# lms-org/trajectory_controller

Measured on AMD Instinct MI355X. Metric: MPC QP solves/sec (horizon N=20, 2 inputs) at 1/2/4/8 MI355X; max|du| vs dlib, higher is better.
Workload: dtype f64; 1 GPU; batch 262144 trajectories per GPU, N=20, 2 inputs, compact (mpcControllerTobi) form, cold start, eps 0.01, max_iter 10000; global_batch=262144, horizon=20, algo=lane_fma, parallelism=batch-sharded x1, batches_in_flight=1, gather=none (1 GPU)

## Files before the change

trajectory_controller_amd/csrc/mpc_internal.h:

```cpp
#pragma once

#include <hip/hip_runtime.h>
#include <stdint.h>

namespace tpc {

constexpr int kWave = 64;

struct Knobs {
    double eps;
    uint32_t max_iter;
    uint32_t smo_iters;
};

struct CompactArgs {
    int64_t n;
    const void *v, *dy, *dphi;
    void *front, *rear;
    int32_t* iters;
    uint32_t* flags;
    const int32_t* work_hint;
    double step, wheelbase;
    double q[2], r[2], lo[2], hi[2];
    int table_key;
// ... 25 lines not shown
struct Workspace {
    void* state;
    uint32_t* ticket;
    unsigned long long* stats;
    int64_t capacity_bytes;
    uint32_t *keys, *rank, *order;
    void* sort_temp;
    size_t sort_temp_bytes;
    hipEvent_t* ev;
    int wave_group = 0;
    int group_lanes = 0;
    int max_waves = 0;
    bool group_pair = false;
    int64_t lanex_below = -1;
    int cu_count = 0;
};

constexpr int kQueueTickets = 16;
constexpr int kQueueTicketStride = 64;
constexpr int64_t kQueueTicketBytes = (int64_t)kQueueTickets * kQueueTicketStride * 4;
constexpr int64_t kWaveQueueMaxInstances = 32768;

constexpr int kAlgoMixed = 101;
constexpr int kAlgoGeneric = 100;
constexpr int kMaxHorizon = 64;
int64_t generic_scratch_bytes(int H, int dtype, int64_t n);
hipError_t generic_compact(int dtype, int H, const CompactArgs& a, const Knobs& k, void* scratch, hipStream_t s);
hipError_t generic_general(int dtype, int I, int H, const GeneralArgs& a, const Knobs& k, void* scratch, hipStream_t s);

size_t sort_temp_bytes(int64_t n);
hipError_t order_begin(void* temp, hipStream_t s);
hipError_t presolve_merge(const uint32_t* queue, const uint32_t* queue_len, int64_t n, const void* sf, const void* sr,
                          const int32_t* si, void* f, void* r, int32_t* it, uint32_t limit, hipStream_t s);
hipError_t presolve_merge_rows(const uint32_t* queue, const uint32_t* queue_len, int64_t n, const void* su, const int32_t* si,
                               void* u, int32_t* it, int rows, int64_t ld, uint32_t limit, hipStream_t s);
const uint32_t* order_queue_len(const void* temp);
hipError_t order_finish(const uint32_t* keys, const uint32_t* rank, uint32_t* order, int64_t n, void* temp,
                        hipStream_t s);

struct RolloutStepArgs {
    int64_t n, ld, ld_out, ld_nlt;
    int I, H, step, steps;
    const void *A, *B, *C;
    void* x;
    void* targets;
// ... 40 lines not shown
```

trajectory_controller_amd/csrc/mpc_lane_inst.hip:

```cpp
#include <cstdint>

#include "mpc_lane.h"
#include "mpc_lanex.h"

#ifndef TPC_LANE_H
#error "compile with -DTPC_LANE_H=<horizon>"
#endif

namespace tpc {

namespace {

constexpr int kH = TPC_LANE_H;

template <class Tag, class Kernel>
inline int pg_grid(Kernel kernel, int block) {
    constexpr int kMaxDev = 64;
    static int cache[kMaxDev] = {0};
    int dev = 0;
    if (hipGetDevice(&dev) != hipSuccess) dev = 0;
    if (dev >= 0 && dev < kMaxDev && cache[dev] > 0) return cache[dev];
    int cus = 256, per_cu = 4;
    hipDeviceProp_t prop;
    if (hipGetDeviceProperties(&prop, dev) == hipSuccess) cus = prop.multiProcessorCount;
    if (hipOccupancyMaxActiveBlocksPerMultiprocessor(&per_cu, kernel, block, 0) != hipSuccess || per_cu < 1)
        per_cu = 1;
    if (per_cu > 4) per_cu = 4;
    if (dev >= 0 && dev < kMaxDev) cache[dev] = cus * per_cu;
    return cus * per_cu;
}
struct TagState {}; struct TagFast {}; struct TagExact {}; struct TagLanex {}; template <int I> struct TagLanexG {};

inline bool wants_state(const CompactArgs&) { return false; }
inline bool wants_state(const GeneralArgs& a) { return a.controls != nullptr || a.v != nullptr; }

template <typename T, int I, class Model, class Args>
hipError_t phase1(const Args& a, const Knobs& k, const Workspace& ws, hipStream_t s) {
    T* recs = (T*)ws.state;
    hipError_t e = hipMemsetAsync(ws.ticket, 0, sizeof(uint32_t), s);
    if (e == hipSuccess) e = hipMemsetAsync(ws.stats, 0, 3 * sizeof(unsigned long long), s);
    if (e == hipSuccess) e = order_begin(ws.sort_temp, s);
    if (e != hipSuccess) return e;
    const int cd_grid = (int)((a.n + kWave - 1) / kWave);
    if (ws.ev) (void)hipEventRecord(ws.ev[0], s);
    hipLaunchKernelGGL((lane_cd_kernel<T, I, kH, Model, Args>), dim3(cd_grid), dim3(kWave), 0, s, a, k, recs,
                       ws.keys, ws.rank, (uint32_t*)ws.sort_temp, ws.stats, wants_state(a) ? 0 : 1);
    e = hipGetLastError();
    if (e != hipSuccess) return e;
    e = order_finish(ws.keys, ws.rank, ws.order, a.n, ws.sort_temp, s);
    if (e != hipSuccess) return e;
    if (ws.ev) (void)hipEventRecord(ws.ev[1], s);
    return hipSuccess;
}
template <typename T, int I, class Model, class Args>
hipError_t phase2(const Args& a, const Knobs& k, const Workspace& ws, hipStream_t s, bool only_if_refused) {
    T* recs = (T*)ws.state;
// ... 68 lines not shown
            if (ws.ev) (void)hipEventRecord(ws.ev[2], s);
            return e;
        }
    }
    e = phase2<T, I, Model, Args>(a, k, ws, s, false);
    if (ws.ev) (void)hipEventRecord(ws.ev[2], s);
    return e;
}

template <typename T, int I, class Model, class Args, int SUBSET = 1>
hipError_t resolve(const Args& a, const Knobs& k, const Workspace& ws, const int32_t* select, const uint32_t* gate, hipStream_t s,
                   double lambda_from = 0.0, const uint32_t* pre_len = nullptr, uint32_t pre_limit = 0u) {
    if (a.n <= 0) return hipSuccess;
    T* recs = (T*)ws.state;
    uint32_t* queue_len = ws.ticket + 1;
    hipError_t e = hipMemsetAsync(ws.ticket, 0, 32, s);
    if (e != hipSuccess) return e;
    const int grid = (int)((a.n + kWave - 1) / kWave);
    hipLaunchKernelGGL((lane_cd_kernel<T, I, kH, Model, Args, SUBSET>), dim3(grid), dim3(kWave), 0, s, a, k, recs, ws.order,
                       (uint32_t*)nullptr, queue_len, ws.stats, 1, select, gate, (T)lambda_from, pre_len, pre_limit);
    if constexpr (std::is_same<Model, CompactModel<T>>::value && sizeof(T) == 8 && LanexPlan<kH>::built) {
        constexpr int ng = LanexPlan<kH>::NG;
        const int64_t need = (a.n + ng - 1) / ng;
        if constexpr (SUBSET == 2) {
            const int64_t solo = (int64_t)pre_limit / ng;
            hipLaunchKernelGGL((lanex_pg_kernel<T, kH, true>), dim3((unsigned)(need < solo ? need : solo)), dim3(kWave), 0, s, a, k,
                               (const T*)recs, (const uint32_t*)ws.order, ws.ticket, ws.stats, (const uint32_t*)queue_len, 1, pre_limit);
            return hipGetLastError();
        }
        const int grid_cap = pg_grid<TagLanex>(lanex_pg_kernel<T, kH>, kWave);
        hipLaunchKernelGGL((lanex_pg_kernel<T, kH>), dim3((unsigned)(need < grid_cap ? need : grid_cap)), dim3(kWave), 0, s, a, k,
// ... 89 lines not shown
```

trajectory_controller_amd/csrc/mpc_sort.hip:

```cpp
#include "mpc_internal.h"

namespace tpc {

namespace {

constexpr int kBins = 1 << 16;

constexpr int kScanBlocks = 64, kScanThreads = 256, kPerThread = kBins / kScanBlocks / kScanThreads;

__global__ __launch_bounds__(kScanThreads) void scan_sums_kernel(const uint32_t* __restrict__ hist,
                                                                 uint32_t* __restrict__ block_sum) {
    __shared__ uint32_t part[kScanThreads / 64];
    const int t = threadIdx.x;
    const int top = kBins - 1 - (blockIdx.x * kScanThreads + t) * kPerThread;
    uint32_t sum = 0;
    for (int j = 0; j < kPerThread; ++j) sum += hist[top - j];
    for (int off = 32; off > 0; off >>= 1) sum += __shfl_down(sum, off);
    if ((t & 63) == 0) part[t >> 6] = sum;
    __syncthreads();
    if (t == 0) {
        uint32_t tot = 0;
        for (int w = 0; w < kScanThreads / 64; ++w) tot += part[w];
        block_sum[blockIdx.x] = tot;
    }
}

__global__ __launch_bounds__(kScanThreads) void scan_apply_kernel(uint32_t* __restrict__ hist,
                                                                  const uint32_t* __restrict__ block_sum) {
    __shared__ uint32_t part[kScanThreads];
    const int t = threadIdx.x;
    const int top = kBins - 1 - (blockIdx.x * kScanThreads + t) * kPerThread;
    uint32_t c[kPerThread], sum = 0;
    for (int j = 0; j < kPerThread; ++j) { c[j] = hist[top - j]; sum += c[j]; }
    part[t] = sum;
    __syncthreads();
    for (int off = 1; off < kScanThreads; off <<= 1) {
        const uint32_t add = t >= off ? part[t - off] : 0u;
        __syncthreads();
        part[t] += add;
        __syncthreads();
    }
    uint32_t base = part[t] - sum;
    for (int b = 0; b < (int)blockIdx.x; ++b) base += block_sum[b];
    for (int j = 0; j < kPerThread; ++j) {
        hist[top - j] = base;
        base += c[j];
    }
}

__global__ void scatter_kernel(const uint32_t* __restrict__ keys, const uint32_t* __restrict__ rank,
                               const uint32_t* __restrict__ base, uint32_t* __restrict__ order, int64_t n) {
    for (int64_t i = (int64_t)blockIdx.x * blockDim.x + threadIdx.x; i < n; i += (int64_t)gridDim.x * blockDim.x)
        order[base[keys[i] >> 16] + rank[i]] = (uint32_t)i;
}

}

size_t sort_temp_bytes(int64_t) { return (size_t)(kBins + kScanBlocks) * sizeof(uint32_t); }

const uint32_t* order_queue_len(const void* temp) { return (const uint32_t*)temp + 127; }

hipError_t order_begin(void* temp, hipStream_t s) {
    return hipMemsetAsync(temp, 0, (size_t)kBins * sizeof(uint32_t), s);
}

hipError_t order_finish(const uint32_t* keys, const uint32_t* rank, uint32_t* order, int64_t n, void* temp,
                        hipStream_t s) {
    uint32_t* hist = (uint32_t*)temp;
    const int block = 256;
    int64_t g = (n + block - 1) / block;
    const unsigned grid = (unsigned)(g < 2048 ? g : 2048);
    uint32_t* block_sum = hist + kBins;
    hipLaunchKernelGGL(scan_sums_kernel, dim3(kScanBlocks), dim3(kScanThreads), 0, s, (const uint32_t*)hist, block_sum);
    hipLaunchKernelGGL(scan_apply_kernel, dim3(kScanBlocks), dim3(kScanThreads), 0, s, hist, (const uint32_t*)block_sum);
    hipLaunchKernelGGL(scatter_kernel, dim3(grid), dim3(block), 0, s, keys, rank, (const uint32_t*)hist, order, n);
    return hipGetLastError();
}

template <typename T>
__global__ void presolve_merge_kernel(const uint32_t* __restrict__ queue, const uint32_t* __restrict__ queue_len,
                                      const T* __restrict__ sf, const T* __restrict__ sr, const int32_t* __restrict__ si,
                                      T* __restrict__ f, T* __restrict__ r, int32_t* __restrict__ it, uint32_t limit) {
    const uint32_t nq = *queue_len;
    if (nq > limit) return;
    for (uint32_t q = blockIdx.x * blockDim.x + threadIdx.x; q < nq; q += gridDim.x * blockDim.x) {
        const uint32_t k = queue[q];
        f[k] = sf[k];
        r[k] = sr[k];
        if (it) it[k] = si[k];
    }
// ... 29 lines not shown
```

trajectory_controller_amd/csrc/mpc_ub.h:

```cpp
#pragma once

#include "mpc_lane.h"
#include "mpc_ub_model.h"
#include "mpc_ub_cd_asm.h"
#include "mpc_queue_key.h"

namespace tpc {

template <typename T, bool EQB> TPC_DEV void ub_set_uniform(ub::Unit<T, EQB>& m, T gscale, const CompactArgs& g) {
    const T q[2] = {(T)g.q[0], (T)g.q[1]}, r[2] = {(T)g.r[0], (T)g.r[1]};
    const T lo[2] = {(T)g.lo[0], (T)g.lo[1]}, hi[2] = {(T)g.hi[0], (T)g.hi[1]};
    m.set_uniform(gscale, q, r, lo, hi);
}

template <typename T, int H> struct UbCdPlan {
    static constexpr bool mirror = 2 * (2 * H * kWave * (int)sizeof(T)) <= 64 * 1024 &&
                                   2 * (2 * H * kWave * (int)sizeof(T)) * 4 * CdOcc<T, H>::value <= 160 * 1024;
    static constexpr bool x_in_lds = mirror && sizeof(T) == 8 && H >= 20;
    static constexpr bool fast = true;
};

template <typename T, int H, bool EQB> struct UbCdAsm {
#ifdef TPC_UB_CD_NO_ASM
    static constexpr bool value = false;
// ... 2 lines not shown
#endif
};

TPC_DEV double cd_ldexp(double x, int e) { return __builtin_ldexp(x, e); }
TPC_DEV float cd_ldexp(float x, int e) { return __builtin_ldexpf(x, e); }

template <typename T, int H, bool EQB>
__global__ __launch_bounds__(64, (CdOcc<T, H>::value)) void ub_cd_kernel(CompactArgs g, Knobs kn, T* __restrict__ recs,
                                                                         uint32_t* __restrict__ keys,
                                                                         uint32_t* __restrict__ key_rank,
                                                                         uint32_t* __restrict__ key_hist,
                                                                         unsigned long long* __restrict__ stats) {
    using P = UbCdPlan<T, H>;
    constexpr int RL = LaneRec<T, H>::kLen;
    constexpr bool MIRROR = P::mirror, XL = P::x_in_lds;
    __shared__ T s_cd[2 * H + (MIRROR ? 2 * H : 1)][kWave];
    T (*const s_iqd)[kWave] = s_cd;
    T (*const s_x)[kWave] = s_cd + 2 * H;
    const int lane = threadIdx.x;
    const int64_t k = (int64_t)blockIdx.x * kWave + lane;
    if (k >= g.n) return;

    ub::Unit<T, EQB> m;
    ub_set_uniform(m, (T)1, g);
    const T ty = ((const T*)g.dy)[k], tphi = ((const T*)g.dphi)[k];
    const T tv = ((const T*)g.v)[k];
    m.set_instance((T)g.step, (T)g.wheelbase, tv, ty, tphi);
    const bool nonfinite = m.nonfinite_inputs(ty, tphi);
    float table_lf = 0.0f;
    if constexpr (sizeof(T) == 8 && H == kQueueKeyH) {
        const float c = queue_key_predict((double)tv, (double)ty, (double)tphi);
        table_lf = (c * c) * (c * c);
    }
    const T q0 = (T)g.q[0], q1 = (T)g.q[1], r0 = (T)g.r[0], r1 = (T)g.r[1];

    T x[XL ? 1 : 2 * H], w[ub::Reverse<T, H>::value ? 1 : 2 * H];
// ... 100 lines not shown
        } else {
#pragma unroll 1
            for (uint32_t it = 0; it < cd_iters; ++it) {
                if (__ballot(!stopped) == 0ull) break;
                iteration(std::true_type{}, it);
            }
        }
    } else {
#pragma unroll 1
        for (uint32_t it = 0; it < cd_iters; ++it) {
            if (__ballot(!stopped) == 0ull) break;
            iteration(std::false_type{}, it);
        }
    }

    T* rec = recs + (int64_t)k * RL;
#pragma unroll
    for (int q = 0; q < 2 * H; ++q) rec[q] = X(q);
    rec[2 * H] = lambda;
    uint64_t meta = (uint64_t)iter;
    if (stopped) meta |= kMetaStopped;
    if (vinit) meta |= kMetaVInit;
    if (nonfinite) meta |= kMetaNonFinite;
    store_meta<T>(rec + 2 * H + 1, meta);
    {
        T il0, il1, beta;
        ub::pg_constants<T>(lambda, m.s0, m.s1, il0, il1, beta);
        T* ex = rec + LaneRec<T, H>::kExtra;
        ex[0] = il0; ex[1] = il1; ex[2] = beta; ex[3] = m.a; ex[4] = m.c; ex[5] = ty; ex[6] = tphi;
    }
    const bool finished = stopped || iter >= kn.max_iter;
    const T lambda_floor = (r0 + r1) * (T)H;
    const bool uninformative = lambda < (T)1.5 * lambda_floor;
    float lf = (float)lambda;
    if constexpr (sizeof(T) == 8 && H == kQueueKeyH) {
        if (g.table_key) lf = table_lf;
    }
    if (g.work_hint) lf = (float)(g.work_hint[k] > 0 ? g.work_hint[k] : 1);
    const uint32_t spread = (uint32_t)k & 127u;
    uint32_t key = __float_as_uint(lf);
    if (finished) key = spread << 16;
    else if (!g.work_hint && uninformative) key = (0x7f00u + spread) << 16;
    else if (!(lf > 0.0f) || key < 0x00800000u) key = 0x00800000u;
    else if (key >= 0x7f000000u) key = 0x7effffffu;
    uint32_t f = 0;
    if (finished) {
        ((T*)g.front)[k] = nonfinite ? (T)0 : m.control(0, X(0));
        ((T*)g.rear)[k] = nonfinite ? (T)0 : m.control(1, X(1));
        if (g.iters) g.iters[k] = (int32_t)iter;
        if (nonfinite) f |= 0x1u;
        if (!stopped) f |= 0x2u;
    }
    raise_flags(g.flags, f);
    keys[k] = key;
    key_rank[k] = atomicAdd(&key_hist[key >> 16], 1u);
}

#ifndef TPC_UB_OCC
#define TPC_UB_OCC 0
#endif
#ifndef TPC_UB_KV
#define TPC_UB_KV -1
#endif
template <typename T, int H> struct UbPlan {
    static constexpr bool D = sizeof(T) == 8;
    static constexpr int words = D ? 2 : 1;
    static constexpr bool reverse = ub::Reverse<T, H>::value;
    static constexpr bool regs = 6 * H * words <= 200 || !D || (reverse && 4 * H * words <= 200);
// ... 238 lines not shown
```

trajectory_controller_amd/csrc/mpc_ub_inst.hip:

```cpp
#include <cstdint>
#include <type_traits>

#include "mpc_ub.h"

#ifndef TPC_UB_H
#error "compile with -DTPC_UB_H=<horizon>"
#endif

namespace tpc {

hipError_t ub_pg_asm_launch(const CompactArgs& a, const Knobs& k, const Workspace& ws, int64_t need, hipStream_t s);
hipError_t ub_pg_asm_launch_h10(const CompactArgs& a, const Knobs& k, const Workspace& ws, int64_t need, hipStream_t s);

namespace {

constexpr int kH = TPC_UB_H;

template <class Tag, class Kernel>
inline int ub_grid(Kernel kernel, int block) {
    constexpr int kMaxDev = 64;
    static int cache[kMaxDev] = {0};
    int dev = 0;
    if (hipGetDevice(&dev) != hipSuccess) dev = 0;
    if (dev >= 0 && dev < kMaxDev && cache[dev] > 0) return cache[dev];
    int cus = 256, per_cu = 4;
    hipDeviceProp_t prop;
    if (hipGetDeviceProperties(&prop, dev) == hipSuccess) cus = prop.multiProcessorCount;
    if (hipOccupancyMaxActiveBlocksPerMultiprocessor(&per_cu, kernel, block, 0) != hipSuccess || per_cu < 1)
        per_cu = 1;
    if (per_cu > 4) per_cu = 4;
    if (dev >= 0 && dev < kMaxDev) cache[dev] = cus * per_cu;
    return cus * per_cu;
}
template <typename T, bool EQB, int MODE> struct TagPg {};

template <typename T, bool EQB>
hipError_t phase1(const CompactArgs& a, const Knobs& k, const Workspace& ws, hipStream_t s) {
    T* recs = (T*)ws.state;
    hipError_t e = hipMemsetAsync(ws.ticket, 0, sizeof(uint32_t), s);
    if (e == hipSuccess) e = hipMemsetAsync(ws.stats, 0, 3 * sizeof(unsigned long long), s);
    if (e == hipSuccess) e = order_begin(ws.sort_temp, s);
    if (e != hipSuccess) return e;
    const int cd_grid = (int)((a.n + kWave - 1) / kWave);
    if (ws.ev) (void)hipEventRecord(ws.ev[0], s);
    hipLaunchKernelGGL((ub_cd_kernel<T, kH, EQB>), dim3(cd_grid), dim3(kWave), 0, s, a, k, recs, ws.keys, ws.rank,
                       (uint32_t*)ws.sort_temp, ws.stats);
    e = hipGetLastError();
    if (e != hipSuccess) return e;
    e = order_finish(ws.keys, ws.rank, ws.order, a.n, ws.sort_temp, s);
    if (e != hipSuccess) return e;
    if (ws.ev) (void)hipEventRecord(ws.ev[1], s);
    return hipSuccess;
}
template <typename T, bool EQB, int MODE>
hipError_t pg_launch(const CompactArgs& a, const Knobs& k, const Workspace& ws, hipStream_t s) {
    constexpr int bt = kWave * UbPlan<T, kH>::occ;
// ... 58 lines not shown
```

trajectory_controller_amd/csrc/tpc_mpc_api.cpp:

```cpp
#include "tpc_mpc_context.h"
#include "tpc_mpc_experimental.h"
#include "auto_table.h"
#include "mpc_queue_key_table.h"
#include "mpc_grad_model.h"
#include "mpc_polish_model.h"
#include "mpc_rollout_newton.h"
#include "mpc_newton_compact.h"
#include "mpc_tangent_model.h"

#include <cmath>
#include <cstdlib>
#include <mutex>
#include <vector>

namespace tpc {
#define TPC_DECL_H(h)                                                                             \
    hipError_t lane_compact_h##h(int, const CompactArgs&, const Knobs&, const Workspace&, hipStream_t); \
    hipError_t lane_general_h##h(int, int, const GeneralArgs&, const Knobs&, const Workspace&, hipStream_t); \
    hipError_t lane_resolve_compact_h##h(const CompactArgs&, const Knobs&, const Workspace&, const int32_t*, const uint32_t*, hipStream_t, double, const uint32_t*, uint32_t); \
    hipError_t lane_presolve_compact_h##h(const CompactArgs&, const Knobs&, const Workspace&, double, uint32_t, hipStream_t); \
    hipError_t lane_resolve_general_h##h(int, const GeneralArgs&, const Knobs&, const Workspace&, const int32_t*, const uint32_t*, hipStream_t, double, const uint32_t*, uint32_t); \
    hipError_t lane_presolve_general_h##h(int, const GeneralArgs&, const Knobs&, const Workspace&, double, uint32_t, hipStream_t); \
    hipError_t wave_compact_h##h(int, const CompactArgs&, const Knobs&, const Workspace&, hipStream_t); \
    hipError_t wave_general_h##h(int, int, const GeneralArgs&, const Knobs&, const Workspace&, hipStream_t); \
// ... 291 lines not shown
        int rc = ensure(h, &h->ws_state, &h->ws_bytes, pad256(generic_scratch_bytes(H, dtype, n)));
        if (rc) return rc;
        ws->state = h->ws_state;
        ws->capacity_bytes = h->ws_bytes;
    }
    if (algo == TPC_MPC_ALGO_WAVE) {
        int rc = ensure(h, &h->ws_state, &h->ws_bytes, pad256(n * 4) + kQueueTicketBytes);
        if (rc) return rc;
        ws->order = (uint32_t*)h->ws_state;
        ws->ticket = (uint32_t*)((char*)h->ws_state + pad256(n * 4));
        ws->capacity_bytes = h->ws_bytes;
    }
    if (algo == TPC_MPC_ALGO_LANE || algo == TPC_MPC_ALGO_LANE_FMA || algo == TPC_MPC_ALGO_GROUP) {
        const int64_t rec_b = pad256(lane_rec_len(H, dtype) * (int64_t)esize(dtype) * n);
        const int64_t col_b = pad256(n * 4);
        const size_t tmp_b = sort_temp_bytes(n);
        int rc = ensure(h, &h->ws_state, &h->ws_bytes, rec_b + 3 * col_b + pad256((int64_t)tmp_b));
        if (rc) return rc;
        char* b = (char*)h->ws_state;
        ws->state = b;
        ws->keys = (uint32_t*)(b + rec_b);
        ws->rank = (uint32_t*)(b + rec_b + col_b);
        ws->order = (uint32_t*)(b + rec_b + 2 * col_b);
        ws->sort_temp = b + rec_b + 3 * col_b;
        ws->sort_temp_bytes = tmp_b;
        ws->capacity_bytes = h->ws_bytes;
    }
    return TPC_MPC_OK;
}

int resolve_reserve(tpc_mpc_context* h, int H, int dtype, int64_t n) { return reserve_lane_workspace(h, H, dtype, n); }
int resolve_workspace(tpc_mpc_context* h, int H, int dtype, int64_t n, Workspace* ws) {
    const bool ev_valid = h->ev_valid;
    const int last_algo = h->last_algo;
    const int rc = prepare_workspace(h, TPC_MPC_ALGO_LANE, H, dtype, n, ws);
    h->ev_valid = ev_valid;
    h->last_algo = last_algo;
    ws->ev = nullptr;
    ws->ticket = h->ws_words + 16;
    ws->stats = (unsigned long long*)(h->ws_words + 18);
    return rc;
}

hipError_t copy_rows(void* dst, int64_t dpitch, const void* src, int64_t spitch, int64_t width, int64_t rows,
                     hipMemcpyKind kind, hipStream_t s) {
    if (rows <= 0 || width <= 0) return hipSuccess;
    if (dpitch == width && spitch == width) return hipMemcpyAsync(dst, src, (size_t)(width * rows), kind, s);
    return hipMemcpy2DAsync(dst, (size_t)dpitch, src, (size_t)spitch, (size_t)width, (size_t)rows, kind, s);
}

int check_general_io(tpc_mpc_context* h, const tpc_mpc_general_io* io, int mem) {
    if (!io) return fail(h, TPC_MPC_ERR_BAD_ARG, "null io");
    if (io->inputs != 1 && io->inputs != 2) return fail(h, TPC_MPC_ERR_BAD_ARG, "inputs must be 1 or 2");
    if (io->n < 0 || io->ld < io->n || io->n > 0x7fffffffll)
        return fail(h, TPC_MPC_ERR_BAD_ARG, "need 0 <= n <= ld, n < 2^31");
// ... 27 lines not shown

int check_compact_model(tpc_mpc_context* h, const tpc_mpc_params* p) {
    if (!(p->weight_y >= 0) || !(p->weight_phi >= 0))
        return fail(h, TPC_MPC_ERR_BAD_WEIGHTS, "min(Q) >= 0 violated (mpc_abstract.h:90-97)");
    if (!(p->weight_steering_front > 0) || !(p->weight_steering_rear > 0))
        return fail(h, TPC_MPC_ERR_BAD_WEIGHTS, "min(R) > 0 violated (mpc_abstract.h:90-97)");
    for (int j = 0; j < 2; ++j)
        if (!(p->upper[j] >= p->lower[j]))
            return fail(h, TPC_MPC_ERR_BAD_BOUNDS, "upper >= lower violated (mpc_abstract.h:90-97)");
    if (!std::isfinite(p->step_size) || !std::isfinite(p->wheelbase) || p->wheelbase == 0)
        return fail(h, TPC_MPC_ERR_BAD_ARG, "step_size / wheelbase must be finite, wheelbase != 0");
    return TPC_MPC_OK;
}

int stream_order_begin(tpc_mpc_context* h, hipStream_t s) {
    if (h->have_last && h->last_stream != s) HIP_TRY(h, hipStreamWaitEvent(s, h->done_ev, 0));
    return TPC_MPC_OK;
}
int stream_order_end(tpc_mpc_context* h, hipStream_t s) {
    HIP_TRY(h, hipEventRecord(h->done_ev, s));
    h->last_stream = s;
    h->have_last = true;
    return TPC_MPC_OK;
}

int finish_flags(tpc_mpc_context* h, uint32_t* flags_out, hipStream_t s) {
    if (!flags_out) return TPC_MPC_OK;
    uint32_t f = 0;
    HIP_TRY(h, hipMemcpyAsync(&f, h->ws_words + 1, sizeof(f), hipMemcpyDeviceToHost, s));
    HIP_TRY(h, hipStreamSynchronize(s));
    *flags_out = f;
    return TPC_MPC_OK;
}

int reserve_lane_workspace(tpc_mpc_context* h, int H, int dtype, int64_t n) {
    const bool ev_valid = h->ev_valid;
    const int last_algo = h->last_algo;
    Workspace ws;
    const int rc = prepare_workspace(h, horizon_specialised(H) ? TPC_MPC_ALGO_LANE : kAlgoGeneric, H, dtype, n, &ws);
    h->ev_valid = ev_valid;
    h->last_algo = last_algo;
    return rc;
}

int context_new(int device, int cu_count, tpc_mpc_context** out) {
    tpc_mpc_context* h = new (std::nothrow) tpc_mpc_context;
    if (!h) return fail(nullptr, TPC_MPC_ERR_ALLOC, "out of host memory");
    h->device = device;
    h->cu_count = cu_count;
    h->device_cu_count = cu_count;
    hipError_t e = hipSetDevice(device);
    if (e == hipSuccess) e = hipMalloc((void**)&h->ws_words, 128);
    if (e == hipSuccess) e = hipMemset(h->ws_words, 0, 128);
    if (e == hipSuccess) e = hipHostMalloc(&h->pin_host, 512, hipHostMallocMapped | hipHostMallocCoherent);
    if (e == hipSuccess) e = hipHostGetDevicePointer(&h->pin_dev, h->pin_host, 0);
    if (e == hipSuccess) e = hipEventCreateWithFlags(&h->done_ev, hipEventDisableTiming);
    if (e != hipSuccess) {
        (void)tpc_mpc_destroy(h);
        return fail(nullptr, TPC_MPC_ERR_HIP, "create: %s", hipGetErrorString(e));
    }
    std::memset(h->pin_host, 0, 512);
    *out = h;
    return TPC_MPC_OK;
}

static double presolve_lambda(const tpc_mpc_params* p);
static int presolve_scratch(tpc_mpc_context* h, int H, int dtype, int64_t n, int64_t side_bytes, Workspace* ws, char** side) {
    const int64_t rec_b = pad256(lane_rec_len(H, dtype) * (int64_t)esize(dtype) * n), col_b = pad256(n * 4);
// ... 4 lines not shown
    if (!h->pre_stream) HIP_TRY(h, hipStreamCreateWithFlags(&h->pre_stream, hipStreamNonBlocking));
    if (!h->pre_fork) HIP_TRY(h, hipEventCreateWithFlags(&h->pre_fork, hipEventDisableTiming));
    if (!h->pre_done) HIP_TRY(h, hipEventCreateWithFlags(&h->pre_done, hipEventDisableTiming));
    char* b = (char*)h->pre;
    std::memset(ws, 0, sizeof(*ws));
    ws->state = b;
    ws->keys = (uint32_t*)(b + rec_b);
    ws->rank = (uint32_t*)(b + rec_b + col_b);
    ws->order = (uint32_t*)(b + rec_b + 2 * col_b);
    ws->sort_temp = b + rec_b + 3 * col_b;
    ws->sort_temp_bytes = tmp_b;
    ws->capacity_bytes = lane_b;
    ws->ev = nullptr;
    ws->lanex_below = h->opt_lanex_below;
    ws->cu_count = h->cu_count;
    ws->ticket = h->ws_words + 24;
    ws->stats = (unsigned long long*)(h->ws_words + 26);
    *side = b + lane_b;
    return TPC_MPC_OK;
}
static bool presolve_share(tpc_mpc_context* h, int64_t n, Presolve* ps) {
    const int simds = (h->device_cu_count > 0 ? h->device_cu_count : 256) * 4;
    const int solo_waves = simds * 7 / 16;
    if (n > (int64_t)solo_waves * 8 * 5) return false;
    ps->limit = (uint32_t)solo_waves * 8u;
    ps->group_waves = simds - solo_waves;
    return true;
}

int general_launch(tpc_mpc_context* h, const tpc_mpc_params* p, const tpc_mpc_general_io* io, hipStream_t s) {
    const int I = io->inputs, H = p->horizon;
    const int64_t n = io->n;
// ... 180 lines not shown
    if (algo < 0) return fail(h, TPC_MPC_ERR_BAD_HORIZON, "the WAVE kernel exists for the specialised horizons with inputs*horizon <= 64 only; use LANE or AUTO");
    CompactArgs a;
    compact_args(h, p, n, v, dy, dphi, front, rear, iters, &a);
    a.work_hint = take_hint(h, n);
    a.table_key = h->opt_queue_key && queue_key_table_applies(p, algo) ? 1 : 0;
    h->last_queue_key = a.work_hint ? kQueueKeyHint : (a.table_key ? kQueueKeyTableUsed : kQueueKeyLambda);
    const bool fix = wants_cap_resolve(p, algo) && a.flags;
    int rc = TPC_MPC_OK;
    if (fix && !a.iters) rc = cap_iters_buffer(h, n, &a.iters);
    if (!rc && fix) rc = resolve_reserve(h, p->horizon, p->dtype, n);
    if (rc) return rc;
    ps->select = a.iters;
    Workspace ws;
    rc = prepare_workspace(h, algo, p->horizon, p->dtype, n, &ws);
    if (rc) return rc;
    hipError_t e = dispatch_compact(algo, p->horizon, p->dtype, a, knobs_of(p), ws, s);
    if (e != hipSuccess) return hip_fail(h, e, "kernel launch");
    if (ps->deferred) return TPC_MPC_OK;
    return presolve_finish(h, p, n, v, dy, dphi, front, rear, iters, s, ps);
}

int compact_launch(tpc_mpc_context* h, const tpc_mpc_params* p, int64_t n, const void* v, const void* dy,
                   const void* dphi, void* front, void* rear, int32_t* iters, hipStream_t s) {
    Presolve ps;
    int rc = presolve_begin(h, p, n, v, dy, dphi, s, &ps);
    if (!rc) rc = compact_launch_ps(h, p, n, v, dy, dphi, front, rear, iters, s, &ps);
    if (rc && ps.on) {
        h->pre_busy = false;
        (void)hipEventRecord(h->pre_done, h->pre_stream);
        (void)hipStreamWaitEvent(s, h->pre_done, 0);
// ... 191 lines not shown
        int rc = check_common(h, p);
        if (rc) return rc;
        rc = check_compact_model(h, p);
        if (rc) return rc;
        if (n < 0 || n > 0x7fffffffll) return fail(h, TPC_MPC_ERR_BAD_ARG, "need 0 <= n < 2^31");
        if (mem != TPC_MPC_HOST && mem != TPC_MPC_DEVICE) return fail(h, TPC_MPC_ERR_BAD_ARG, "bad memory kind");
        if (n == 0) { if (flags_out) *flags_out = 0; return TPC_MPC_OK; }
        if (!v || !delta_y || !delta_phi || !steering_front || !steering_rear)
            return fail(h, TPC_MPC_ERR_BAD_ARG, "null batch pointer");
        HIP_TRY(h, hipSetDevice(h->device));
        hipStream_t s = (hipStream_t)stream;
        const int64_t es = (int64_t)esize(p->dtype);
        StreamOrderScope order(h, s);
        rc = order.begin();
        if (rc) return rc;
        HIP_TRY(h, hipMemsetAsync(h->ws_words + 1, 0, sizeof(uint32_t), s));
        if (mem == TPC_MPC_DEVICE) {
            rc = compact_launch(h, p, n, v, delta_y, delta_phi, steering_front, steering_rear, iters, s);
            if (rc) return rc;
        } else {
            const int64_t col = pad256(n * es), icol = pad256(n * 4);
            rc = ensure(h, &h->stage, &h->stage_bytes, 5 * col + icol);
            if (rc) return rc;
            char* b = (char*)h->stage;
            HIP_TRY(h, hipMemcpyAsync(b, v, n * es, hipMemcpyHostToDevice, s));
            HIP_TRY(h, hipMemcpyAsync(b + col, delta_y, n * es, hipMemcpyHostToDevice, s));
            HIP_TRY(h, hipMemcpyAsync(b + 2 * col, delta_phi, n * es, hipMemcpyHostToDevice, s));
            int32_t* d_it = iters ? (int32_t*)(b + 5 * col) : nullptr;
            rc = compact_launch(h, p, n, b, b + col, b + 2 * col, b + 3 * col, b + 4 * col, d_it, s);
            if (rc) return rc;
            HIP_TRY(h, hipMemcpyAsync(steering_front, b + 3 * col, n * es, hipMemcpyDeviceToHost, s));
// ... 1328 lines not shown
        HIP_TRY(h, hipSetDevice(h->device));
        hipStream_t s = (hipStream_t)stream;
        const int64_t n = t->n;
        StreamOrderScope order(h, s);
        rc = order.begin();
        if (rc) return rc;
        const int64_t col = pad256(n * 8);
        rc = ensure(h, &h->roll, &h->roll_bytes, 3 * col);
        if (rc) return rc;
        char* b = (char*)h->roll;
        FollowArgs fa = follow_args(t, lookup_x, lookup_y, lookup_n);
        fa.v_out = (double*)b; fa.ysoll_out = (double*)(b + col); fa.phisoll_out = (double*)(b + 2 * col);
        fa.target_speed = target_speed; fa.target_distance = target_distance;
        hipError_t e = launch_traj_point(fa, s);
        if (e != hipSuccess) return hip_fail(h, e, "traj_point launch");
        HIP_TRY(h, hipMemsetAsync(h->ws_words + 1, 0, sizeof(uint32_t), s));
        rc = compact_launch(h, p, n, fa.v_out, fa.ysoll_out, fa.phisoll_out, steering_front, steering_rear, iters, s);
        if (rc) return rc;
        e = launch_follow_post(n, target_speed, steering_front, steering_rear, s);
        if (e != hipSuccess) return hip_fail(h, e, "follow_post launch");
        rc = order.end();
        if (rc) return rc;
        return finish_flags(h, flags_out, s);
    });
}

int tpc_mpc_follow_batch_horizon(tpc_mpc_handle h, const tpc_mpc_params* p, const tpc_mpc_trajectories* t,
                                 const float* step_spacing, const float* lookup_x, const float* lookup_y,
                                 int32_t lookup_n, double* steering_front, double* steering_rear,
                                 float* target_speed, float* target_distance, double* targets_out,
                                 int32_t* iters, uint32_t* flags_out, void* stream) {
// ... 245 lines not shown
```

trajectory_controller_amd/csrc/tpc_mpc_comm.cpp:

```cpp
#include "tpc_mpc_context.h"
#include "tpc_mpc_experimental.h"

#include <dlfcn.h>
#include <cstdlib>
#include <mutex>
#include <rccl/rccl.h>

namespace tpc {

struct Comm {
    ncclComm_t comm = nullptr;
    int rank = 0, world = 1;
};

namespace {

struct Rccl {
    void* lib = nullptr;
    decltype(&ncclGetUniqueId) GetUniqueId = nullptr;
    decltype(&ncclCommInitRank) CommInitRank = nullptr;
    decltype(&ncclCommDestroy) CommDestroy = nullptr;
    decltype(&ncclAllGather) AllGather = nullptr;
    decltype(&ncclBroadcast) Broadcast = nullptr;
    decltype(&ncclGroupStart) GroupStart = nullptr;
// ... 266 lines not shown
        char* front = (char*)steering_front_all;
        char* rear = (char*)steering_rear_all;
        const bool exchange = world > 1 || h->comm;
        const bool staged = split == TPC_MPC_SPLIT_INTERLEAVED && exchange;
        const int64_t cap = interleaved_cap(n_total, world);
        char *sf = nullptr, *sr = nullptr;
        if (staged) {
            rc = ensure(h, &h->gather, &h->gather_bytes, 2 * pad256(world * cap * es));
            if (rc) return rc;
            sf = (char*)h->gather;
            sr = sf + pad256(world * cap * es);
        }
        StreamOrderScope order(h, s);
        rc = order.begin();
        if (rc) return rc;
        HIP_TRY(h, hipMemsetAsync(h->ws_words + 1, 0, sizeof(uint32_t), s));
        if (count > 0) {
            char* of = staged ? sf + rank * cap * es : front + first * es;
            char* orr = staged ? sr + rank * cap * es : rear + first * es;
            rc = compact_launch(h, p, count, v_shard, delta_y_shard, delta_phi_shard, of, orr, iters_shard, s);
            if (rc) return rc;
        }
        if (exchange) {
            Rccl* r = rccl();
            if (!r) return fail(h, TPC_MPC_ERR_COMM, "RCCL is not available in this process: %s", g_rccl.why);
            XOp ops[kMaxOps];
            const int n_ops = exchange_plan(n_total, world, rank, split, h->comm_test_ragged, ops, kMaxOps);
            GroupScope group(r);
            RCCL_TRY(h, r, group.begin());
            rc = run_plan(h, r, ops, n_ops, staged ? sf : front, (int)es, s);
            if (rc) return rc;
// ... 143 lines not shown
```

trajectory_controller_amd/csrc/tpc_mpc_context.h:

```cpp
#pragma once

#include "../../include/tpc_mpc.h"

#include <hip/hip_runtime.h>

#include <cstdarg>
#include <cstdio>
#include <cstring>
#include <exception>
#include <new>

#include "mpc_internal.h"

namespace tpc {
struct OneShot;
int context_new(int device, int cu_count, tpc_mpc_context** out);
struct Comm;
}

constexpr size_t kTpcErrLen = 512;

struct tpc_mpc_context {
    int device = 0;
    int cu_count = 0;
    int device_cu_count = 0;
    char err[kTpcErrLen] = "";
    void* ws_state = nullptr;
    int64_t ws_bytes = 0;
    uint32_t* ws_words = nullptr;
    void* stage = nullptr;
    int64_t stage_bytes = 0;
    void* roll = nullptr;
    int64_t roll_bytes = 0;
    void* cap_iters = nullptr;
    int64_t cap_iters_bytes = 0;
    void* grad_ws = nullptr;
    int64_t grad_ws_bytes = 0;
    void* newton = nullptr;
    int64_t newton_bytes = 0;
    void* newton_fb = nullptr;
    int64_t newton_fb_bytes = 0;
    void* pre = nullptr;
    int64_t pre_bytes = 0;
    hipStream_t pre_stream = nullptr;
// ... 88 lines not shown
    hipError_t e = hipMalloc(buf, (size_t)grow);
    if (e != hipSuccess) {
        *buf = nullptr;
        (void)hipGetLastError();
        return fail(h, TPC_MPC_ERR_ALLOC, "hipMalloc of %lld bytes: %s", (long long)grow, hipGetErrorString(e));
    }
    *have = grow;
    return TPC_MPC_OK;
}

int check_common(tpc_mpc_context* h, const tpc_mpc_params* p, bool host_ok = false);
int check_compact_model(tpc_mpc_context* h, const tpc_mpc_params* p);
int stream_order_begin(tpc_mpc_context* h, hipStream_t s);
int stream_order_end(tpc_mpc_context* h, hipStream_t s);
int finish_flags(tpc_mpc_context* h, uint32_t* flags_out, hipStream_t s);
struct StreamOrderScope {
    tpc_mpc_context* h;
    hipStream_t s;
    bool armed = false;
    StreamOrderScope(tpc_mpc_context* hh, hipStream_t ss) : h(hh), s(ss) {}
    int begin() { const int rc = stream_order_begin(h, s); armed = rc == 0; return rc; }
    int end() { armed = false; return stream_order_end(h, s); }
    ~StreamOrderScope() { if (armed) (void)stream_order_end(h, s); }
};
int general_launch(tpc_mpc_context* h, const tpc_mpc_params* p, const tpc_mpc_general_io* io, hipStream_t s);
int check_general_device_io(tpc_mpc_context* h, const tpc_mpc_general_io* io);
int compact_launch(tpc_mpc_context* h, const tpc_mpc_params* p, int64_t n, const void* v, const void* dy,
                   const void* dphi, void* front, void* rear, int32_t* iters, hipStream_t s);
struct Presolve {
    bool on = false;
// ... 29 lines not shown
```

trajectory_controller_amd/csrc/tpc_mpc_mixed.hip:

```cpp
#include "tpc_mpc_context.h"

namespace tpc {

namespace {

constexpr int kBinsMax = 8;

struct MixedBins {
    int nb;
    int horizon[kBinsMax];
};

__device__ __forceinline__ int bin_of(const MixedBins& b, int h) {
    int r = b.nb;
#pragma unroll
    for (int i = 0; i < kBinsMax - 1; ++i)
        if (i < b.nb && b.horizon[i] == h) r = i;
    return r;
}

__global__ __launch_bounds__(256) void mixed_bin_kernel(const int32_t* __restrict__ horizons, int64_t n, MixedBins bins,
                                                        uint32_t* __restrict__ counts, uint32_t* __restrict__ slot) {
    const int64_t k = (int64_t)blockIdx.x * blockDim.x + threadIdx.x;
    const bool live = k < n;
// ... 87 lines not shown
    bool any_group = false;
    for (int i = 0; i < bins.nb; ++i) {
        if (!hc[i]) continue;
        ++live;
        any_group = any_group || group_applicable(h, p, bins.horizon[i]);
    }
    if (!h->fork_ev) HIP_TRY(h, hipEventCreateWithFlags(&h->fork_ev, hipEventDisableTiming));
    if (any_group || live == 1) {
        int last = -1;
        for (int i = 0; i < bins.nb; ++i)
            if (hc[i]) last = i;
        Presolve ps;
        tpc_mpc_params ql = *p;
        ql.horizon = bins.horizon[last];
        const int64_t ol = ho[last];
        int rc = presolve_begin(h, &ql, hc[last], gv + ol, gdy + ol, gdphi + ol, s, &ps);
        ps.deferred = true;
        auto bail = [&](int code) {
            if (ps.on) { (void)hipEventRecord(h->pre_done, h->pre_stream); (void)hipStreamWaitEvent(s, h->pre_done, 0); h->pre_busy = false; }
            return code;
        };
        if (rc) return bail(rc);
        for (int i = 0; i < bins.nb; ++i) {
            if (!hc[i]) continue;
            tpc_mpc_params q = *p;
            q.horizon = bins.horizon[i];
            const int64_t o = ho[i];
            if (i == last) rc = compact_launch_ps(h, &q, hc[i], gv + o, gdy + o, gdphi + o, gfront + o, grear + o, d_iters ? giters + o : nullptr, s, &ps);
            else rc = compact_launch(h, &q, hc[i], gv + o, gdy + o, gdphi + o, gfront + o, grear + o, d_iters ? giters + o : nullptr, s);
            if (rc) return bail(rc);
        }
// ... 29 lines not shown
                if (e != hipSuccess) {
                    if (ks) (void)hipStreamDestroy(ks);
                    (void)tpc_mpc_destroy(kid);
                    join();
                    return hip_fail(h, e, "mixed batch: child stream / event");
                }
                h->kids[i] = kid; h->kid_stream[i] = ks; h->kid_done[i] = ke;
            }
            tpc_mpc_context* kid = h->kids[i];
            kid->opt_wave_group = h->opt_wave_group;
            kid->opt_group_lanes = h->opt_group_lanes;
            hipStream_t ks = h->kid_stream[i];
            hipError_t e = hipStreamWaitEvent(ks, h->fork_ev, 0);
            if (e != hipSuccess) { join(); return hip_fail(h, e, "mixed batch: fork"); }
            forked[i] = true;
            e = hipMemsetAsync(kid->ws_words + 1, 0, sizeof(uint32_t), ks);
            if (e != hipSuccess) { join(); return hip_fail(h, e, "mixed batch: flag word"); }
            int rc = compact_launch(kid, &q, hc[i], gv + o, gdy + o, gdphi + o, gfront + o, grear + o,
                                    d_iters ? giters + o : nullptr, ks);
            if (rc) { join(); return fail(h, rc, "mixed batch, horizon %d: %s", q.horizon, kid->err); }
            hipLaunchKernelGGL(mixed_or_flags_kernel, dim3(1), dim3(1), 0, ks, h->ws_words + 1, (const uint32_t*)(kid->ws_words + 1));
            e = hipGetLastError();
            if (e != hipSuccess) { join(); return hip_fail(h, e, "mixed batch: flags"); }
        }
        {
            hipError_t e = hipSuccess;
            for (int i = 0; i < bins.nb && e == hipSuccess; ++i) {
                if (!forked[i]) continue;
                e = hipEventRecord(h->kid_done[i], h->kid_stream[i]);
                if (e == hipSuccess) e = hipStreamWaitEvent(s, h->kid_done[i], 0);
            }
            if (e != hipSuccess) { join(); return hip_fail(h, e, "mixed batch: join"); }
        }
// ... 78 lines not shown
```

Baseline: 61.97 million solves/s.

## Merge per-call memsets into one, fuse sort scan kernels, stage records via LDS

Moves the sort histogram into the small per-handle words buffer so a single memset per call clears the flag word, ticket, stats and histogram, and later phases skip their own memsets when that has happened. The two-kernel block-sum scan becomes one kernel in which each block recomputes the totals of the blocks above it from vectorised loads. When x lives in LDS, the lane kernel assembles its records in shared memory and writes them out coalesced in 16-byte pairs instead of strided per-lane stores. The aim is fewer launches and memsets per call plus better store coalescing, at the cost of redundant scan reads and extra zeroed-state bookkeeping.

```diff
diff --git a/trajectory_controller_amd/csrc/mpc_internal.h b/trajectory_controller_amd/csrc/mpc_internal.h
--- a/trajectory_controller_amd/csrc/mpc_internal.h
+++ b/trajectory_controller_amd/csrc/mpc_internal.h
@@ -63,6 +63,7 @@
     bool group_pair = false;
     int64_t lanex_below = -1;
     int cu_count = 0;
+    bool zeroed = false;
 };
 
 constexpr int kQueueTickets = 16;
@@ -78,6 +79,7 @@
 hipError_t generic_general(int dtype, int I, int H, const GeneralArgs& a, const Knobs& k, void* scratch, hipStream_t s);
 
 size_t sort_temp_bytes(int64_t n);
+size_t sort_count_bytes();
 hipError_t order_begin(void* temp, hipStream_t s);
 hipError_t presolve_merge(const uint32_t* queue, const uint32_t* queue_len, int64_t n, const void* sf, const void* sr,
                           const int32_t* si, void* f, void* r, int32_t* it, uint32_t limit, hipStream_t s);
diff --git a/trajectory_controller_amd/csrc/mpc_lane_inst.hip b/trajectory_controller_amd/csrc/mpc_lane_inst.hip
--- a/trajectory_controller_amd/csrc/mpc_lane_inst.hip
+++ b/trajectory_controller_amd/csrc/mpc_lane_inst.hip
@@ -37,9 +37,12 @@
 template <typename T, int I, class Model, class Args>
 hipError_t phase1(const Args& a, const Knobs& k, const Workspace& ws, hipStream_t s) {
     T* recs = (T*)ws.state;
-    hipError_t e = hipMemsetAsync(ws.ticket, 0, sizeof(uint32_t), s);
-    if (e == hipSuccess) e = hipMemsetAsync(ws.stats, 0, 3 * sizeof(unsigned long long), s);
-    if (e == hipSuccess) e = order_begin(ws.sort_temp, s);
+    hipError_t e = hipSuccess;
+    if (!ws.zeroed) {
+        e = hipMemsetAsync(ws.ticket, 0, sizeof(uint32_t), s);
+        if (e == hipSuccess) e = hipMemsetAsync(ws.stats, 0, 3 * sizeof(unsigned long long), s);
+        if (e == hipSuccess) e = order_begin(ws.sort_temp, s);
+    }
     if (e != hipSuccess) return e;
     const int cd_grid = (int)((a.n + kWave - 1) / kWave);
     if (ws.ev) (void)hipEventRecord(ws.ev[0], s);
@@ -138,7 +141,7 @@
     if (a.n <= 0) return hipSuccess;
     T* recs = (T*)ws.state;
     uint32_t* queue_len = ws.ticket + 1;
-    hipError_t e = hipMemsetAsync(ws.ticket, 0, 32, s);
+    hipError_t e = ws.zeroed ? hipSuccess : hipMemsetAsync(ws.ticket, 0, 32, s);
     if (e != hipSuccess) return e;
     const int grid = (int)((a.n + kWave - 1) / kWave);
     hipLaunchKernelGGL((lane_cd_kernel<T, I, kH, Model, Args, SUBSET>), dim3(grid), dim3(kWave), 0, s, a, k, recs, ws.order,
diff --git a/trajectory_controller_amd/csrc/mpc_sort.hip b/trajectory_controller_amd/csrc/mpc_sort.hip
--- a/trajectory_controller_amd/csrc/mpc_sort.hip
+++ b/trajectory_controller_amd/csrc/mpc_sort.hip
@@ -7,28 +7,21 @@
 constexpr int kBins = 1 << 16;
 
 constexpr int kScanBlocks = 64, kScanThreads = 256, kPerThread = kBins / kScanBlocks / kScanThreads;
+static_assert(kPerThread == 4, "one 16-byte vector per thread and block of the counts above");
 
-__global__ __launch_bounds__(kScanThreads) void scan_sums_kernel(const uint32_t* __restrict__ hist,
-                                                                 uint32_t* __restrict__ block_sum) {
-    __shared__ uint32_t part[kScanThreads / 64];
+__global__ __launch_bounds__(kScanThreads) void scan_kernel(const uint32_t* __restrict__ hist, uint32_t* __restrict__ first) {
+    __shared__ uint32_t part[kScanThreads];
+    __shared__ uint32_t above_part[kScanThreads / 64];
     const int t = threadIdx.x;
-    const int top = kBins - 1 - (blockIdx.x * kScanThreads + t) * kPerThread;
-    uint32_t sum = 0;
-    for (int j = 0; j < kPerThread; ++j) sum += hist[top - j];
-    for (int off = 32; off > 0; off >>= 1) sum += __shfl_down(sum, off);
-    if ((t & 63) == 0) part[t >> 6] = sum;
-    __syncthreads();
-    if (t == 0) {
-        uint32_t tot = 0;
-        for (int w = 0; w < kScanThreads / 64; ++w) tot += part[w];
-        block_sum[blockIdx.x] = tot;
+    const uint4* above = (const uint4*)(hist + kBins - (int)blockIdx.x * kScanThreads * kPerThread);
+    uint32_t pre = 0;
+#pragma unroll 8
+    for (int b = 0; b < (int)blockIdx.x; ++b) {
+        const uint4 q = above[b * kScanThreads + t];
+        pre += (q.x + q.y) + (q.z + q.w);
     }
-}
-
-__global__ __launch_bounds__(kScanThreads) void scan_apply_kernel(uint32_t* __restrict__ hist,
-                                                                  const uint32_t* __restrict__ block_sum) {
-    __shared__ uint32_t part[kScanThreads];
-    const int t = threadIdx.x;
+    for (int off = 32; off > 0; off >>= 1) pre += __shfl_down(pre, off);
+    if ((t & 63) == 0) above_part[t >> 6] = pre;
     const int top = kBins - 1 - (blockIdx.x * kScanThreads + t) * kPerThread;
     uint32_t c[kPerThread], sum = 0;
     for (int j = 0; j < kPerThread; ++j) { c[j] = hist[top - j]; sum += c[j]; }
@@ -41,9 +34,9 @@
         __syncthreads();
     }
     uint32_t base = part[t] - sum;
-    for (int b = 0; b < (int)blockIdx.x; ++b) base += block_sum[b];
+    for (int w = 0; w < kScanThreads / 64; ++w) base += above_part[w];
     for (int j = 0; j < kPerThread; ++j) {
-        hist[top - j] = base;
+        first[top - j] = base;
         base += c[j];
     }
 }
@@ -56,9 +49,11 @@
 
 }
 
-size_t sort_temp_bytes(int64_t) { return (size_t)(kBins + kScanBlocks) * sizeof(uint32_t); }
+size_t sort_temp_bytes(int64_t) { return (size_t)(2 * kBins) * sizeof(uint32_t); }
 
-const uint32_t* order_queue_len(const void* temp) { return (const uint32_t*)temp + 127; }
+const uint32_t* order_queue_len(const void* temp) { return (const uint32_t*)temp + kBins + 127; }
+
+size_t sort_count_bytes() { return (size_t)kBins * sizeof(uint32_t); }
 
 hipError_t order_begin(void* temp, hipStream_t s) {
     return hipMemsetAsync(temp, 0, (size_t)kBins * sizeof(uint32_t), s);
@@ -70,10 +65,9 @@
     const int block = 256;
     int64_t g = (n + block - 1) / block;
     const unsigned grid = (unsigned)(g < 2048 ? g : 2048);
-    uint32_t* block_sum = hist + kBins;
-    hipLaunchKernelGGL(scan_sums_kernel, dim3(kScanBlocks), dim3(kScanThreads), 0, s, (const uint32_t*)hist, block_sum);
-    hipLaunchKernelGGL(scan_apply_kernel, dim3(kScanBlocks), dim3(kScanThreads), 0, s, hist, (const uint32_t*)block_sum);
-    hipLaunchKernelGGL(scatter_kernel, dim3(grid), dim3(block), 0, s, keys, rank, (const uint32_t*)hist, order, n);
+    uint32_t* first = hist + kBins;
+    hipLaunchKernelGGL(scan_kernel, dim3(kScanBlocks), dim3(kScanThreads), 0, s, (const uint32_t*)hist, first);
+    hipLaunchKernelGGL(scatter_kernel, dim3(grid), dim3(block), 0, s, keys, rank, (const uint32_t*)first, order, n);
     return hipGetLastError();
 }
 
diff --git a/trajectory_controller_amd/csrc/mpc_ub.h b/trajectory_controller_amd/csrc/mpc_ub.h
--- a/trajectory_controller_amd/csrc/mpc_ub.h
+++ b/trajectory_controller_amd/csrc/mpc_ub.h
@@ -40,12 +40,13 @@
     using P = UbCdPlan<T, H>;
     constexpr int RL = LaneRec<T, H>::kLen;
     constexpr bool MIRROR = P::mirror, XL = P::x_in_lds;
-    __shared__ T s_cd[2 * H + (MIRROR ? 2 * H : 1)][kWave];
+    __shared__ alignas(16) T s_cd[2 * H + (MIRROR ? 2 * H : 1)][kWave];
     T (*const s_iqd)[kWave] = s_cd;
     T (*const s_x)[kWave] = s_cd + 2 * H;
     const int lane = threadIdx.x;
-    const int64_t k = (int64_t)blockIdx.x * kWave + lane;
-    if (k >= g.n) return;
+    const bool mine = (int64_t)blockIdx.x * kWave + lane < g.n;
+    if constexpr (!XL) { if (!mine) return; }
+    const int64_t k = mine ? (int64_t)blockIdx.x * kWave + lane : g.n - 1;
 
     ub::Unit<T, EQB> m;
     ub_set_uniform(m, (T)1, g);
@@ -176,9 +177,24 @@
         }
     }
 
-    T* rec = recs + (int64_t)k * RL;
-#pragma unroll
-    for (int q = 0; q < 2 * H; ++q) rec[q] = X(q);
+    T xv[XL ? 2 * H : 1];
+    T* rec;
+    if constexpr (XL) {
+#pragma unroll
+        for (int q = 0; q < 2 * H; ++q) xv[q] = s_x[q][lane];
+        __syncthreads();
+        static_assert(kWave * RL <= (int)(sizeof(s_cd) / sizeof(T)) && RL % 2 == 0, "the wavefront's records fit the LDS array, in 16-byte pairs");
+        rec = &s_cd[0][0] + lane * RL;
+        if constexpr (RL > LaneRec<T, H>::kExtra + LaneRec<T, H>::kExtras) rec[RL - 1] = (T)0;
+    } else {
+        rec = recs + (int64_t)k * RL;
+    }
+    T x0, x1;
+    if constexpr (XL) { x0 = xv[0]; x1 = xv[1]; } else { x0 = X(0); x1 = X(1); }
+#pragma unroll
+    for (int q = 0; q < 2 * H; ++q) {
+        if constexpr (XL) rec[q] = xv[q]; else rec[q] = X(q);
+    }
     rec[2 * H] = lambda;
     uint64_t meta = (uint64_t)iter;
     if (stopped) meta |= kMetaStopped;
@@ -191,6 +207,16 @@
         T* ex = rec + LaneRec<T, H>::kExtra;
         ex[0] = il0; ex[1] = il1; ex[2] = beta; ex[3] = m.a; ex[4] = m.c; ex[5] = ty; ex[6] = tphi;
     }
+    if constexpr (XL) {
+        __syncthreads();
+        const int64_t first = (int64_t)blockIdx.x * kWave;
+        const int count = g.n - first < kWave ? (int)(g.n - first) : kWave;
+        typedef T Pair __attribute__((ext_vector_type(2)));
+        const Pair* from = (const Pair*)&s_cd[0][0];
+        Pair* to = (Pair*)(recs + first * RL);
+#pragma unroll 5
+        for (int p = lane; p < count * (RL / 2); p += kWave) to[p] = from[p];
+    }
     const bool finished = stopped || iter >= kn.max_iter;
     const T lambda_floor = (r0 + r1) * (T)H;
     const bool uninformative = lambda < (T)1.5 * lambda_floor;
@@ -206,14 +232,15 @@
     else if (!(lf > 0.0f) || key < 0x00800000u) key = 0x00800000u;
     else if (key >= 0x7f000000u) key = 0x7effffffu;
     uint32_t f = 0;
-    if (finished) {
-        ((T*)g.front)[k] = nonfinite ? (T)0 : m.control(0, X(0));
-        ((T*)g.rear)[k] = nonfinite ? (T)0 : m.control(1, X(1));
+    if (finished && mine) {
+        ((T*)g.front)[k] = nonfinite ? (T)0 : m.control(0, x0);
+        ((T*)g.rear)[k] = nonfinite ? (T)0 : m.control(1, x1);
         if (g.iters) g.iters[k] = (int32_t)iter;
         if (nonfinite) f |= 0x1u;
         if (!stopped) f |= 0x2u;
     }
     raise_flags(g.flags, f);
+    if (!mine) return;
     keys[k] = key;
     key_rank[k] = atomicAdd(&key_hist[key >> 16], 1u);
 }
diff --git a/trajectory_controller_amd/csrc/mpc_ub_inst.hip b/trajectory_controller_amd/csrc/mpc_ub_inst.hip
--- a/trajectory_controller_amd/csrc/mpc_ub_inst.hip
+++ b/trajectory_controller_amd/csrc/mpc_ub_inst.hip
@@ -37,9 +37,12 @@
 template <typename T, bool EQB>
 hipError_t phase1(const CompactArgs& a, const Knobs& k, const Workspace& ws, hipStream_t s) {
     T* recs = (T*)ws.state;
-    hipError_t e = hipMemsetAsync(ws.ticket, 0, sizeof(uint32_t), s);
-    if (e == hipSuccess) e = hipMemsetAsync(ws.stats, 0, 3 * sizeof(unsigned long long), s);
-    if (e == hipSuccess) e = order_begin(ws.sort_temp, s);
+    hipError_t e = hipSuccess;
+    if (!ws.zeroed) {
+        e = hipMemsetAsync(ws.ticket, 0, sizeof(uint32_t), s);
+        if (e == hipSuccess) e = hipMemsetAsync(ws.stats, 0, 3 * sizeof(unsigned long long), s);
+        if (e == hipSuccess) e = order_begin(ws.sort_temp, s);
+    }
     if (e != hipSuccess) return e;
     const int cd_grid = (int)((a.n + kWave - 1) / kWave);
     if (ws.ev) (void)hipEventRecord(ws.ev[0], s);
diff --git a/trajectory_controller_amd/csrc/tpc_mpc_api.cpp b/trajectory_controller_amd/csrc/tpc_mpc_api.cpp
--- a/trajectory_controller_amd/csrc/tpc_mpc_api.cpp
+++ b/trajectory_controller_amd/csrc/tpc_mpc_api.cpp
@@ -329,16 +329,15 @@
     if (algo == TPC_MPC_ALGO_LANE || algo == TPC_MPC_ALGO_LANE_FMA || algo == TPC_MPC_ALGO_GROUP) {
         const int64_t rec_b = pad256(lane_rec_len(H, dtype) * (int64_t)esize(dtype) * n);
         const int64_t col_b = pad256(n * 4);
-        const size_t tmp_b = sort_temp_bytes(n);
-        int rc = ensure(h, &h->ws_state, &h->ws_bytes, rec_b + 3 * col_b + pad256((int64_t)tmp_b));
+        int rc = ensure(h, &h->ws_state, &h->ws_bytes, rec_b + 3 * col_b);
         if (rc) return rc;
         char* b = (char*)h->ws_state;
         ws->state = b;
         ws->keys = (uint32_t*)(b + rec_b);
         ws->rank = (uint32_t*)(b + rec_b + col_b);
         ws->order = (uint32_t*)(b + rec_b + 2 * col_b);
-        ws->sort_temp = b + rec_b + 3 * col_b;
-        ws->sort_temp_bytes = tmp_b;
+        ws->sort_temp = h->ws_words + kWsWordsFront;
+        ws->sort_temp_bytes = sort_temp_bytes(n);
         ws->capacity_bytes = h->ws_bytes;
     }
     return TPC_MPC_OK;
@@ -354,6 +353,8 @@
     ws->ev = nullptr;
     ws->ticket = h->ws_words + 16;
     ws->stats = (unsigned long long*)(h->ws_words + 18);
+    ws->zeroed = h->zeroed_second;
+    h->zeroed_second = false;
     return rc;
 }
 
@@ -411,13 +412,27 @@
 }
 
 int stream_order_begin(tpc_mpc_context* h, hipStream_t s) {
+    h->zeroed_first = h->zeroed_second = false;
     if (h->have_last && h->last_stream != s) HIP_TRY(h, hipStreamWaitEvent(s, h->done_ev, 0));
     return TPC_MPC_OK;
 }
 int stream_order_end(tpc_mpc_context* h, hipStream_t s) {
+    h->zeroed_first = h->zeroed_second = false;
     HIP_TRY(h, hipEventRecord(h->done_ev, s));
     h->last_stream = s;
     h->have_last = true;
+    return TPC_MPC_OK;
+}
+
+int reset_call_words(tpc_mpc_context* h, const tpc_mpc_params* p, int64_t n, hipStream_t s) {
+    const int algo = pick_algo(h, p->algo, 2, p->horizon, n, p->dtype, fma_usable(p));
+    if (algo != TPC_MPC_ALGO_LANE && algo != TPC_MPC_ALGO_LANE_FMA && algo != TPC_MPC_ALGO_GROUP) {
+        h->zeroed_first = h->zeroed_second = false;
+        HIP_TRY(h, hipMemsetAsync(h->ws_words + 1, 0, sizeof(uint32_t), s));
+        return TPC_MPC_OK;
+    }
+    HIP_TRY(h, hipMemsetAsync(h->ws_words, 0, kWsWordsFront * sizeof(uint32_t) + sort_count_bytes(), s));
+    h->zeroed_first = h->zeroed_second = true;
     return TPC_MPC_OK;
 }
 
@@ -447,8 +462,9 @@
     h->cu_count = cu_count;
     h->device_cu_count = cu_count;
     hipError_t e = hipSetDevice(device);
-    if (e == hipSuccess) e = hipMalloc((void**)&h->ws_words, 128);
-    if (e == hipSuccess) e = hipMemset(h->ws_words, 0, 128);
+    const size_t words_b = kWsWordsFront * sizeof(uint32_t) + sort_temp_bytes(0) + 8 * sizeof(uint32_t);
+    if (e == hipSuccess) e = hipMalloc((void**)&h->ws_words, words_b);
+    if (e == hipSuccess) e = hipMemset(h->ws_words, 0, words_b);
     if (e == hipSuccess) e = hipHostMalloc(&h->pin_host, 512, hipHostMallocMapped | hipHostMallocCoherent);
     if (e == hipSuccess) e = hipHostGetDevicePointer(&h->pin_dev, h->pin_host, 0);
     if (e == hipSuccess) e = hipEventCreateWithFlags(&h->done_ev, hipEventDisableTiming);
@@ -483,8 +499,8 @@
     ws->ev = nullptr;
     ws->lanex_below = h->opt_lanex_below;
     ws->cu_count = h->cu_count;
-    ws->ticket = h->ws_words + 24;
-    ws->stats = (unsigned long long*)(h->ws_words + 26);
+    ws->ticket = h->ws_words + kWsWordsFront + sort_temp_bytes(0) / sizeof(uint32_t);
+    ws->stats = (unsigned long long*)(ws->ticket + 2);
     *side = b + lane_b;
     return TPC_MPC_OK;
 }
@@ -695,6 +711,8 @@
     Workspace ws;
     rc = prepare_workspace(h, algo, p->horizon, p->dtype, n, &ws);
     if (rc) return rc;
+    ws.zeroed = h->zeroed_first && ws.sort_temp != nullptr;
+    h->zeroed_first = false;
     hipError_t e = dispatch_compact(algo, p->horizon, p->dtype, a, knobs_of(p), ws, s);
     if (e != hipSuccess) return hip_fail(h, e, "kernel launch");
     if (ps->deferred) return TPC_MPC_OK;
@@ -916,7 +934,8 @@
         StreamOrderScope order(h, s);
         rc = order.begin();
         if (rc) return rc;
-        HIP_TRY(h, hipMemsetAsync(h->ws_words + 1, 0, sizeof(uint32_t), s));
+        rc = reset_call_words(h, p, n, s);
+        if (rc) return rc;
         if (mem == TPC_MPC_DEVICE) {
             rc = compact_launch(h, p, n, v, delta_y, delta_phi, steering_front, steering_rear, iters, s);
             if (rc) return rc;
@@ -2275,7 +2294,8 @@
         fa.target_speed = target_speed; fa.target_distance = target_distance;
         hipError_t e = launch_traj_point(fa, s);
         if (e != hipSuccess) return hip_fail(h, e, "traj_point launch");
-        HIP_TRY(h, hipMemsetAsync(h->ws_words + 1, 0, sizeof(uint32_t), s));
+        rc = reset_call_words(h, p, n, s);
+        if (rc) return rc;
         rc = compact_launch(h, p, n, fa.v_out, fa.ysoll_out, fa.phisoll_out, steering_front, steering_rear, iters, s);
         if (rc) return rc;
         e = launch_follow_post(n, target_speed, steering_front, steering_rear, s);
diff --git a/trajectory_controller_amd/csrc/tpc_mpc_comm.cpp b/trajectory_controller_amd/csrc/tpc_mpc_comm.cpp
--- a/trajectory_controller_amd/csrc/tpc_mpc_comm.cpp
+++ b/trajectory_controller_amd/csrc/tpc_mpc_comm.cpp
@@ -304,7 +304,8 @@
         StreamOrderScope order(h, s);
         rc = order.begin();
         if (rc) return rc;
-        HIP_TRY(h, hipMemsetAsync(h->ws_words + 1, 0, sizeof(uint32_t), s));
+        rc = reset_call_words(h, p, count, s);
+        if (rc) return rc;
         if (count > 0) {
             char* of = staged ? sf + rank * cap * es : front + first * es;
             char* orr = staged ? sr + rank * cap * es : rear + first * es;
diff --git a/trajectory_controller_amd/csrc/tpc_mpc_context.h b/trajectory_controller_amd/csrc/tpc_mpc_context.h
--- a/trajectory_controller_amd/csrc/tpc_mpc_context.h
+++ b/trajectory_controller_amd/csrc/tpc_mpc_context.h
@@ -28,6 +28,7 @@
     void* ws_state = nullptr;
     int64_t ws_bytes = 0;
     uint32_t* ws_words = nullptr;
+    bool zeroed_first = false, zeroed_second = false;
     void* stage = nullptr;
     int64_t stage_bytes = 0;
     void* roll = nullptr;
@@ -146,6 +147,8 @@
 int stream_order_begin(tpc_mpc_context* h, hipStream_t s);
 int stream_order_end(tpc_mpc_context* h, hipStream_t s);
 int finish_flags(tpc_mpc_context* h, uint32_t* flags_out, hipStream_t s);
+int reset_call_words(tpc_mpc_context* h, const tpc_mpc_params* p, int64_t n, hipStream_t s);
+constexpr int kWsWordsFront = 32;
 struct StreamOrderScope {
     tpc_mpc_context* h;
     hipStream_t s;
diff --git a/trajectory_controller_amd/csrc/tpc_mpc_mixed.hip b/trajectory_controller_amd/csrc/tpc_mpc_mixed.hip
--- a/trajectory_controller_amd/csrc/tpc_mpc_mixed.hip
+++ b/trajectory_controller_amd/csrc/tpc_mpc_mixed.hip
@@ -125,7 +125,13 @@
         tpc_mpc_params ql = *p;
         ql.horizon = bins.horizon[last];
         const int64_t ol = ho[last];
-        int rc = presolve_begin(h, &ql, hc[last], gv + ol, gdy + ol, gdphi + ol, s, &ps);
+        int first = 0;
+        while (first < last && !hc[first]) ++first;
+        tpc_mpc_params qf = *p;
+        qf.horizon = bins.horizon[first];
+        int rc = reset_call_words(h, &qf, hc[first], s);
+        if (rc) return rc;
+        rc = presolve_begin(h, &ql, hc[last], gv + ol, gdy + ol, gdphi + ol, s, &ps);
         ps.deferred = true;
         auto bail = [&](int code) {
             if (ps.on) { (void)hipEventRecord(h->pre_done, h->pre_stream); (void)hipStreamWaitEvent(s, h->pre_done, 0); h->pre_busy = false; }
@@ -185,9 +191,9 @@
             hipError_t e = hipStreamWaitEvent(ks, h->fork_ev, 0);
             if (e != hipSuccess) { join(); return hip_fail(h, e, "mixed batch: fork"); }
             forked[i] = true;
-            e = hipMemsetAsync(kid->ws_words + 1, 0, sizeof(uint32_t), ks);
-            if (e != hipSuccess) { join(); return hip_fail(h, e, "mixed batch: flag word"); }
-            int rc = compact_launch(kid, &q, hc[i], gv + o, gdy + o, gdphi + o, gfront + o, grear + o,
+            int rc = reset_call_words(kid, &q, hc[i], ks);
+            if (rc) { join(); return fail(h, rc, "mixed batch: flag word: %s", kid->err); }
+            rc = compact_launch(kid, &q, hc[i], gv + o, gdy + o, gdphi + o, gfront + o, grear + o,
                                     d_iters ? giters + o : nullptr, ks);
             if (rc) { join(); return fail(h, rc, "mixed batch, horizon %d: %s", q.horizon, kid->err); }
             hipLaunchKernelGGL(mixed_or_flags_kernel, dim3(1), dim3(1), 0, ks, h->ws_words + 1, (const uint32_t*)(kid->ws_words + 1));
```

After: 62.19 million solves/s, median of 6. Within noise of the previous version (+0.4%).
